# tiberiu44/TTS-Cube

Measured on AMD Instinct MI355X. Metric: audio samples/sec (HiFi-GAN vocoder inference), higher is better.
Workload: dtype f32 (split fp16 hi/lo x3 MFMA, fp32 accumulate)

## Files before the change

### ttscube_amd/csrc/conv1d.hip

```cpp
#include <cmath>
#include <cstdlib>
#include <type_traits>

#include "common.hpp"
#include "conv_kernels.hpp"

namespace ttsc {

template <int C, int K, int D>
__global__ __launch_bounds__(256, 2) void conv_f16x3_wide_kernel(ConvArgs a) {
    extern __shared__ __attribute__((aligned(16))) char smem_raw[];
    constexpr int WM = 2, WN = 2;
    constexpr int MI = 2, NJ = 4, NT = WN * NJ * 32;
    constexpr int SPAN = NT + (K - 1) * D;
    constexpr int SPANP = (SPAN + 63) & ~63;
    constexpr int BUFSZ = 4 * SPAN + 2;
    constexpr int NCHUNK = C / 16, COTN = C / 32;
    constexpr int AITEMS = WM * MI * 2 * 64;
    half8* Xp = reinterpret_cast<half8*>(smem_raw);
    half8* Aw = Xp + 2 * BUFSZ;
    const int tid = threadIdx.x, lane = tid & 63, wave = tid >> 6;
    const int wm = wave / WN, wn = wave % WN;
    const int half = lane >> 5, l31 = lane & 31;
    const int b = blockIdx.z;
    const int q0 = blockIdx.x * NT;
    const int lin = a.in_len ? a.in_len[b] : a.Lin;
    if (a.out_len && q0 >= a.out_len[b]) return;
    const int cotg = blockIdx.y * (WM * MI);
#ifdef TTSC_ABLATE
    const unsigned wg_lin = blockIdx.x + gridDim.x * (blockIdx.y + gridDim.y * blockIdx.z);
#endif
    TTSC_STAMP(a, wg_lin, 0);
    TTSC_STAMP_HWID(a, wg_lin, 15);

    f32x16 acc[MI][NJ];
    const float* ai_first = a.acc_init ? (a.resid ? a.resid : (a.accumulate ? a.y : nullptr)) : nullptr;
    const float* ai_second = (a.acc_init && a.resid && a.accumulate) ? a.y : nullptr;
    const unsigned ai_L = (unsigned)a.Lout;
    const unsigned ai_row0 = ((unsigned)b * a.Cout + (cotg + wm * MI) * 32 + 4 * half) * ai_L;
    const int ai_qw = q0 + wn * (NJ * 32) + l31;
    auto acc_load_first = [&](int i) __attribute__((always_inline)) {
        if (ai_first) {
#pragma unroll
            for (int n = 0; n < NJ; ++n) {
                const int q = ai_qw + n * 32;
                const unsigned o = ai_row0 + (unsigned)(i * 32) * ai_L + (unsigned)(q < a.Lout ? q : 0);
#pragma unroll
                for (int g = 0; g < 4; ++g) {
                    unsigned og = o + (unsigned)(8 * g) * ai_L;
#pragma unroll
                    for (int e = 0; e < 4; ++e) {
                        acc[i][n][4 * g + e] = ai_first[og];
                        og += ai_L;
                    }
                }
            }
        } else {
#pragma unroll
            for (int n = 0; n < NJ; ++n)
#pragma unroll
                for (int r = 0; r < 16; ++r) acc[i][n][r] = 0.f;
        }
    };
    auto acc_init_finish = [&]() __attribute__((always_inline)) {
        const float inv = 1.f / a.w_unscale;
        if (ai_second) {
#pragma unroll
            for (int i = 0; i < MI; ++i)
#pragma unroll
                for (int n0 = 0; n0 < NJ; n0 += 2) {
                    float t[2][16];
#pragma unroll
                    for (int n = 0; n < 2; ++n) {
                        const int q = ai_qw + (n0 + n) * 32;
                        const unsigned o = ai_row0 + (unsigned)(i * 32) * ai_L + (unsigned)(q < a.Lout ? q : 0);
#pragma unroll
                        for (int r = 0; r < 16; ++r) t[n][r] = ai_second[o + (unsigned)((r & 3) + 8 * (r >> 2)) * ai_L];
                    }
#pragma unroll
                    for (int n = 0; n < 2; ++n)
#pragma unroll
                        for (int r = 0; r < 16; ++r) acc[i][n0 + n][r] += t[n][r];
                }
        }
        if (a.bias) {
#pragma unroll
            for (int i = 0; i < MI; ++i) {
                float bv[16];
#pragma unroll
                for (int r = 0; r < 16; ++r) bv[r] = a.bias[(cotg + wm * MI + i) * 32 + (r & 3) + 8 * (r >> 2) + 4 * half];
#pragma unroll
                for (int n = 0; n < NJ; ++n)
#pragma unroll
                    for (int r = 0; r < 16; ++r) acc[i][n][r] += bv[r];
            }
        }
#pragma unroll
        for (int i = 0; i < MI; ++i)
#pragma unroll
            for (int n = 0; n < NJ; ++n)
#pragma unroll
                for (int r = 0; r < 16; ++r) acc[i][n][r] *= inv;
    };
    if (a.acc_init) {
    } else if (a.epi_prefetch && a.bias && (a.resid || a.accumulate)) {
        const float inv = 1.f / a.w_unscale;
#pragma unroll
        for (int i = 0; i < MI; ++i)
#pragma unroll
            for (int r = 0; r < 16; ++r) {
                const float bv = a.bias[(cotg + wm * MI + i) * 32 + (r & 3) + 8 * (r >> 2) + 4 * half] * inv;
#pragma unroll
                for (int j = 0; j < NJ; ++j) acc[i][j][r] = bv;
            }
    } else {
#pragma unroll
        for (int i = 0; i < MI; ++i)
#pragma unroll
            for (int j = 0; j < NJ; ++j)
#pragma unroll
                for (int r = 0; r < 16; ++r) acc[i][j][r] = 0.f;
    }

    const float* xb = a.x + (size_t)b * C * a.Lin;
    const int lo = q0 - D * ((K - 1) / 2);
    const half8* wsrc = reinterpret_cast<const half8*>(a.wph) + (size_t)cotg * 128 + lane;
    if (a.skew) {
        const unsigned lin_id = blockIdx.x + gridDim.x * (blockIdx.y + gridDim.y * blockIdx.z);
        if (lin_id >= 256u && lin_id < 512u)
            for (int z = 0; z < a.skew; ++z) __builtin_amdgcn_s_sleep(127);
    }

    auto stage_A = [&](int c, int j, int slot) __attribute__((always_inline)) {
        if (TTSC_DBG(a, 8)) return;
        const half8* wj = wsrc + (size_t)(j * NCHUNK + c) * (COTN * 128);
#pragma unroll
        for (int i = 0; i < AITEMS / 64 / 4; ++i) {
            const int blk = wave + i * 4;
            __builtin_amdgcn_global_load_lds((const __attribute__((address_space(1))) void*)(wj + blk * 64),
                                             (__attribute__((address_space(3))) void*)(Aw + slot * AITEMS + blk * 64), 16, 0, 0);
        }
    };

    constexpr int XIT = (2 * SPANP + 255) / 256;
    static_assert(XIT <= K, "one staging item per tap");
    float xr[XIT][8];
    unsigned xoff[XIT];
    int xslot[XIT];
    bool xok[XIT];
#pragma unroll
    for (int e = 0; e < XIT; ++e) {
        const int i = tid + e * 256;
        const int h = i >= SPANP ? 1 : 0;
        const int p = i - h * SPANP;
        const int pos = lo + p;
        xok[e] = pos >= 0 && pos < lin;
        int pc = pos > lin - 1 ? lin - 1 : pos;
        pc = pc < 0 ? 0 : pc;
        xoff[e] = (unsigned)(h * 8 * a.Lin + pc);
        xslot[e] = (p < SPAN && i < 2 * SPANP) ? (h * 2) * SPAN + p : 4 * SPAN;
    }
    auto x_issue_item = [&](int e, int c) __attribute__((always_inline)) {
        const float* rc = xb + (size_t)(c * 16) * a.Lin;
#pragma unroll
        for (int ch = 0; ch < 8; ++ch) xr[e][ch] = rc[(size_t)ch * a.Lin + xoff[e]];
    };
    auto x_commit_item = [&](int e, half8* buf) __attribute__((always_inline)) {
        typedef unsigned u32x4 __attribute__((ext_vector_type(4)));
        u32x4 uh, ul;
#pragma unroll
        for (int ch = 0; ch < 8; ch += 2) {
            float v0 = xok[e] ? xr[e][ch] * a.in_scale : 0.f, v1 = xok[e] ? xr[e][ch + 1] * a.in_scale : 0.f;
            v0 = fmaxf(v0, v0 * a.in_slope);
            v1 = fmaxf(v1, v1 * a.in_slope);
            unsigned h, l;
            split2_f16(v0, v1, h, l);
            uh[ch >> 1] = h;
            ul[ch >> 1] = l;
        }
        const half8 vh = __builtin_bit_cast(half8, uh), vl = __builtin_bit_cast(half8, ul);
        buf[xslot[e]] = vh;
        buf[xslot[e] + (xslot[e] < 4 * SPAN ? SPAN : 1)] = vl;
    };

    const half8* xbase = Xp + (unsigned)((half * 2) * SPAN + wn * (NJ * 32) + l31);
    const half8* abase = Aw + (unsigned)(wm * (MI * 128) + lane);
    auto chunk = [&](int c, auto buf_tag, auto par_tag) __attribute__((always_inline)) {
        constexpr int BUF = decltype(buf_tag)::value;
        constexpr int PAR = decltype(par_tag)::value;
        half8* nxt = Xp + (1 - BUF) * BUFSZ;
#pragma unroll
        for (int j = 0; j < K; ++j) {
            const int slot = (PAR + j) & 1;
            if (j + 1 < K)
                stage_A(c, j + 1, slot ^ 1);
            else
                stage_A(c + 1 < NCHUNK ? c + 1 : c, 0, slot ^ 1);
            __builtin_amdgcn_sched_barrier(0);
            half8 ah[MI], al[MI], bh[NJ], bl[NJ];
#pragma unroll
            for (int i = 0; i < MI; ++i) {
                ah[i] = abase[slot * AITEMS + i * 128];
                al[i] = abase[slot * AITEMS + i * 128 + 64];
            }
#pragma unroll
            for (int n = 0; n < NJ; ++n) {
                bh[n] = xbase[BUF * BUFSZ + j * D + n * 32];
                bl[n] = xbase[BUF * BUFSZ + SPAN + j * D + n * 32];
            }
            const int e = K - 1 - j;
            if (e < XIT && !TTSC_DBG(a, 1)) {
                x_commit_item(e, nxt);
                x_issue_item(e, c + 2 < NCHUNK ? c + 2 : NCHUNK - 1);
            }
#pragma unroll
            for (int i = 0; i < MI; ++i)
#pragma unroll
                for (int n = 0; n < NJ; ++n) acc[i][n] = __builtin_amdgcn_mfma_f32_32x32x16_f16(al[i], bh[n], acc[i][n], 0, 0, 0);
#pragma unroll
            for (int i = 0; i < MI; ++i)
#pragma unroll
                for (int n = 0; n < NJ; ++n) acc[i][n] = __builtin_amdgcn_mfma_f32_32x32x16_f16(ah[i], bl[n], acc[i][n], 0, 0, 0);
#pragma unroll
            for (int i = 0; i < MI; ++i)
#pragma unroll
                for (int n = 0; n < NJ; ++n) acc[i][n] = __builtin_amdgcn_mfma_f32_32x32x16_f16(ah[i], bh[n], acc[i][n], 0, 0, 0);
            __builtin_amdgcn_sched_barrier(0);
            if (!TTSC_DBG(a, 2)) __syncthreads();
        }
    };

    stage_A(0, 0, 0);
#pragma unroll
    for (int e = 0; e < XIT; ++e) x_issue_item(e, 0);
    if (a.acc_init) {
        __builtin_amdgcn_sched_barrier(0);
        acc_load_first(0);
        __builtin_amdgcn_sched_barrier(0);
    }
#pragma unroll
    for (int e = 0; e < XIT; ++e) x_commit_item(e, Xp);
#pragma unroll
    for (int e = 0; e < XIT; ++e) x_issue_item(e, 1);
    if (a.acc_init) {
        __builtin_amdgcn_sched_barrier(0);
#pragma unroll
        for (int i = 1; i < MI; ++i) acc_load_first(i);
        acc_init_finish();
    }
    __syncthreads();
    TTSC_STAMP(a, wg_lin, 1);
    for (int c = 0; c < NCHUNK; c += 2) {
        chunk(c, std::integral_constant<int, 0>(), std::integral_constant<int, 0>());
        chunk(c + 1, std::integral_constant<int, 1>(), std::integral_constant<int, (K & 1)>());
    }
// ... 308 lines not shown
                const int ci = c0 + c < a.Cin ? c0 + c : a.Cin - 1;
                const float* row = xb + (size_t)ci * a.Lin;
#pragma unroll
                for (int k = 0; k < PER; ++k) {
                    int pos = lo + tid + k * 256;
                    pos = pos < 0 ? 0 : (pos > a.Lin - 1 ? a.Lin - 1 : pos);
                    v[c][k] = row[pos];
                }
            }
#pragma unroll
            for (int c = 0; c < CH; ++c)
#pragma unroll
                for (int k = 0; k < PER; ++k) {
                    const int p = tid + k * 256, pos = lo + p;
                    float t = v[c][k] * a.in_scale;
                    t = fmaxf(t, t * a.in_slope);
                    if (p < NT + 2 * HALO) xs[c][p] = (c0 + c < a.Cin && pos >= 0 && pos < lin) ? t : 0.f;
                }
        }
        __syncthreads();
        const int nc = a.Cin - c0 < CH ? a.Cin - c0 : CH;
        for (int c = 0; c < nc; ++c) {
            float w[20];
#pragma unroll
            for (int v4 = 0; v4 < 5; ++v4) {
                const f32x4 t = *reinterpret_cast<const f32x4*>(&xs[c][4 * tid + 4 * v4]);
                w[4 * v4] = t[0]; w[4 * v4 + 1] = t[1]; w[4 * v4 + 2] = t[2]; w[4 * v4 + 3] = t[3];
            }
            const float* wk = ws + (c0 + c) * K;
#pragma unroll
            for (int j = 0; j < 16; ++j) {
                if (j < K) {
                    const float wj = wk[j];
#pragma unroll
                    for (int e = 0; e < 4; ++e) acc[e] = fmaf(wj, w[e + j], acc[e]);
                }
            }
        }
    }
    const float bv = a.bias ? a.bias[0] : 0.f;
    float* yb = a.y + (size_t)b * a.Lout;
    const float* rb = a.resid ? a.resid + (size_t)b * a.Lout : nullptr;
    const int q = q0 + 4 * tid;
    float res[4];
#pragma unroll
    for (int e = 0; e < 4; ++e) {
        const bool ok = q + e < a.Lout;
        float t = (acc[e] + bv + (rb && ok ? rb[q + e] : 0.f)) * a.out_scale;
        t = apply_act(t, a.out_act);
        res[e] = t + (a.accumulate && ok ? yb[q + e] : 0.f);
    }
    if (a.nf_flag) {
        bool bad = false;
#pragma unroll
        for (int e = 0; e < 4; ++e) bad = bad || (q + e < a.Lout && !(fabsf(res[e]) <= 3.0e38f));
        if (bad) atomicOr(a.nf_flag, 1u);
    }
    if (q + 3 < a.Lout && (((uintptr_t)(yb + q)) & 15) == 0) {
        const f32x4 o = {res[0], res[1], res[2], res[3]};
        *reinterpret_cast<f32x4*>(yb + q) = o;
    } else {
#pragma unroll
        for (int e = 0; e < 4; ++e)
            if (q + e < a.Lout) yb[q + e] = res[e];
    }
}

template <int MI, int NJ, int TMAX>
static int launch_f16_t(const ConvArgs& a, int B, hipStream_t s) {
    constexpr int NT = 4 * NJ * 32;
    constexpr int MT = MI * 32;
    dim3 grid((unsigned)ceil_div(a.q_cnt, NT), (unsigned)(a.CoutP / MT), (unsigned)B);
    const size_t lds = (size_t)a.span_pad * 4 * 16 + (size_t)a.ntaps * MI * 2 * 64 * 16;
    if (int rc = ensure_full_lds((const void*)conv_f16x3_kernel<MI, NJ, TMAX>)) return rc;
    hipLaunchKernelGGL((conv_f16x3_kernel<MI, NJ, TMAX>), grid, dim3(256), lds, s, a);
    hipError_t e = hipGetLastError();
    if (e != hipSuccess) {
        set_error("conv_f16x3_kernel launch failed: %s", hipGetErrorString(e));
        return TTSC_EHIP;
    }
    return TTSC_OK;
}

template <int C, int K, int D>
static int launch_f16_wide(const ConvArgs& a0, int B, hipStream_t s) {
    constexpr int NT = 256;
    constexpr int SPAN = NT + (K - 1) * D;
    dim3 grid((unsigned)ceil_div(a0.Lout, NT), (unsigned)(C / 128), (unsigned)B);
    ConvArgs a = a0;
    static const int skew_env = getenv("TTSC_CONV_SKEW") ? atoi(getenv("TTSC_CONV_SKEW")) : 0;
    a.skew = ((size_t)grid.x * grid.y * grid.z >= 1024) ? skew_env : 0;
    static const int epi_env = getenv("TTSC_CONV_EPI_PREFETCH") ? atoi(getenv("TTSC_CONV_EPI_PREFETCH")) : 1;
    a.epi_prefetch = (epi_env && !a.gate && a.out_act == TTSC_ACT_NONE && a.Cout == C && (size_t)B * C * a.Lout < (1ull << 32)) ? 1 : 0;
    constexpr size_t lds = (size_t)2 * (4 * SPAN + 2) * 16 + (size_t)2 * (2 * 2 * 2 * 64) * 16;
    if (int rc = ensure_full_lds((const void*)conv_f16x3_wide_kernel<C, K, D>)) return rc;
    hipLaunchKernelGGL((conv_f16x3_wide_kernel<C, K, D>), grid, dim3(256), lds, s, a);
    hipError_t e = hipGetLastError();
    if (e != hipSuccess) {
        set_error("conv_f16x3_wide_kernel launch failed: %s", hipGetErrorString(e));
        return TTSC_EHIP;
    }
    return TTSC_OK;
}


template <int CIN, int J, int MI, int NJ>
__global__ __launch_bounds__(256, 2) void conv_f16x3_tall_kernel(ConvArgs a) {
    extern __shared__ __attribute__((aligned(16))) char smem_raw[];
    constexpr int WM = 2, WN = 2, NT = WN * NJ * 32;
    constexpr int SPAN = NT + (J - 1);
    constexpr int SPANP = (SPAN + 63) & ~63;
    constexpr int BUFSZ = 4 * SPAN + 2;
    constexpr int NCHUNK = CIN / 16;
    constexpr int AITEMS = WM * MI * 2 * 64;
    static_assert(J % 2 == 0 && NCHUNK % 2 == 0, "slot parity: an even number of taps per chunk, chunks in pairs");
    half8* Xp = reinterpret_cast<half8*>(smem_raw);
    half8* Aw = Xp + 2 * BUFSZ;
    const int tid = threadIdx.x, lane = tid & 63, wave = tid >> 6;
    const int wm = wave / WN, wn = wave % WN;
    const int half = lane >> 5, l31 = lane & 31;
    int bx, by, bz;
    if (a.swz_nx > 0) {
        const unsigned id = blockIdx.x, xcd = id & 7u, u = id >> 3;
        by = (int)(u % (unsigned)a.swz_ny);
        const unsigned t = (u / (unsigned)a.swz_ny) * 8u + xcd;
        bx = (int)(t % (unsigned)a.swz_nx);
        bz = (int)(t / (unsigned)a.swz_nx);
        if (bz >= a.fold_B) return;
    } else {
        bx = blockIdx.x, by = blockIdx.y, bz = blockIdx.z;
    }
    const int b = bz;
    const int q0 = a.q_lo + bx * NT;
    const int lin = a.in_len ? a.in_len[b] : a.Lin;
    if (a.out_len && (long)q0 * a.out_stride + a.out_off >= a.out_len[b]) return;
    const int cotg = by * (WM * MI);
    const int cotN = a.CoutP >> 5;

    f32x16 acc[MI][NJ];
#pragma unroll
    for (int i = 0; i < MI; ++i)
#pragma unroll
        for (int j = 0; j < NJ; ++j)
#pragma unroll
            for (int r = 0; r < 16; ++r) acc[i][j][r] = 0.f;

    const float* xb = a.x + (size_t)b * CIN * a.Lin;
    const int lo = q0 - (J - 1);
    const half8* wsrc = reinterpret_cast<const half8*>(a.wph) + (size_t)cotg * 128 + lane;
    auto stage_A = [&](int c, int j, int slot) __attribute__((always_inline)) {
        const half8* wj = wsrc + (size_t)(j * NCHUNK + c) * ((size_t)cotN * 128);
#pragma unroll
        for (int i = 0; i < AITEMS / 64 / 4; ++i) {
            const int blk = wave + i * 4;
            __builtin_amdgcn_global_load_lds((const __attribute__((address_space(1))) void*)(wj + blk * 64),
                                             (__attribute__((address_space(3))) void*)(Aw + slot * AITEMS + blk * 64), 16, 0, 0);
        }
    };
    constexpr int XIT = (2 * SPANP + 255) / 256;
    static_assert(XIT <= J, "one staging item per tap");
    float xr[XIT][8];
    unsigned xoff[XIT];
    int xslot[XIT];
    bool xok[XIT];
#pragma unroll
    for (int e = 0; e < XIT; ++e) {
        const int i = tid + e * 256;
        const int h = i >= SPANP ? 1 : 0;
        const int p = i - h * SPANP;
        const int pos = lo + p;
        xok[e] = pos >= 0 && pos < lin;
        int pc = pos > lin - 1 ? lin - 1 : pos;
        pc = pc < 0 ? 0 : pc;
        xoff[e] = (unsigned)(h * 8 * a.Lin + pc);
        xslot[e] = (p < SPAN && i < 2 * SPANP) ? (h * 2) * SPAN + p : 4 * SPAN;
    }
    auto x_issue_item = [&](int e, int c) __attribute__((always_inline)) {
        const float* rc = xb + (size_t)(c * 16) * a.Lin;
#pragma unroll
        for (int ch = 0; ch < 8; ++ch) xr[e][ch] = rc[(size_t)ch * a.Lin + xoff[e]];
    };
    auto x_commit_item = [&](int e, half8* buf) __attribute__((always_inline)) {
        typedef unsigned u32x4 __attribute__((ext_vector_type(4)));
        u32x4 uh, ul;
#pragma unroll
        for (int ch = 0; ch < 8; ch += 2) {
            float v0 = xok[e] ? xr[e][ch] * a.in_scale : 0.f, v1 = xok[e] ? xr[e][ch + 1] * a.in_scale : 0.f;
            v0 = fmaxf(v0, v0 * a.in_slope);
            v1 = fmaxf(v1, v1 * a.in_slope);
            unsigned h, l;
            split2_f16(v0, v1, h, l);
            uh[ch >> 1] = h;
            ul[ch >> 1] = l;
        }
        const half8 vh = __builtin_bit_cast(half8, uh), vl = __builtin_bit_cast(half8, ul);
        buf[xslot[e]] = vh;
        buf[xslot[e] + (xslot[e] < 4 * SPAN ? SPAN : 1)] = vl;
    };
    const half8* xbase = Xp + (unsigned)((half * 2) * SPAN + wn * (NJ * 32) + l31);
    const half8* abase = Aw + (unsigned)(wm * (MI * 128) + lane);
    auto chunk = [&](int c, auto buf_tag) __attribute__((always_inline)) {
        constexpr int BUF = decltype(buf_tag)::value;
        half8* nxt = Xp + (1 - BUF) * BUFSZ;
#pragma unroll
        for (int j = 0; j < J; ++j) {
            const int slot = j & 1;
            if (j + 1 < J)
                stage_A(c, j + 1, slot ^ 1);
            else
                stage_A(c + 1 < NCHUNK ? c + 1 : c, 0, slot ^ 1);
            __builtin_amdgcn_sched_barrier(0);
            half8 ah[MI], al[MI], bh[NJ], bl[NJ];
#pragma unroll
            for (int i = 0; i < MI; ++i) {
                ah[i] = abase[slot * AITEMS + i * 128];
                al[i] = abase[slot * AITEMS + i * 128 + 64];
            }
#pragma unroll
            for (int n = 0; n < NJ; ++n) {
                bh[n] = xbase[BUF * BUFSZ + (J - 1 - j) + n * 32];
                bl[n] = xbase[BUF * BUFSZ + SPAN + (J - 1 - j) + n * 32];
            }
            const int e = J - 1 - j;
            if (e < XIT) {
                x_commit_item(e, nxt);
                x_issue_item(e, c + 2 < NCHUNK ? c + 2 : NCHUNK - 1);
            }
#pragma unroll
            for (int i = 0; i < MI; ++i)
#pragma unroll
                for (int n = 0; n < NJ; ++n) acc[i][n] = __builtin_amdgcn_mfma_f32_32x32x16_f16(al[i], bh[n], acc[i][n], 0, 0, 0);
#pragma unroll
            for (int i = 0; i < MI; ++i)
#pragma unroll
                for (int n = 0; n < NJ; ++n) acc[i][n] = __builtin_amdgcn_mfma_f32_32x32x16_f16(ah[i], bl[n], acc[i][n], 0, 0, 0);
#pragma unroll
            for (int i = 0; i < MI; ++i)
#pragma unroll
                for (int n = 0; n < NJ; ++n) acc[i][n] = __builtin_amdgcn_mfma_f32_32x32x16_f16(ah[i], bh[n], acc[i][n], 0, 0, 0);
            __builtin_amdgcn_sched_barrier(0);
            __syncthreads();
        }
    };
    stage_A(0, 0, 0);
#pragma unroll
    for (int e = 0; e < XIT; ++e) x_issue_item(e, 0);
#pragma unroll
    for (int e = 0; e < XIT; ++e) x_commit_item(e, Xp);
#pragma unroll
    for (int e = 0; e < XIT; ++e) x_issue_item(e, 1);
    __syncthreads();
    for (int c = 0; c < NCHUNK; c += 2) {
        chunk(c, std::integral_constant<int, 0>());
        chunk(c + 1, std::integral_constant<int, 1>());
    }
    const int q_hi = a.q_lo + a.q_cnt;
#pragma unroll
    for (int i = 0; i < MI; ++i) {
#pragma unroll
        for (int n = 0; n < NJ; ++n) {
            const int q = q0 + wn * (NJ * 32) + n * 32 + l31;
            int cb = (cotg + wm * MI + i) * 32;
            const int r = cb / a.vphase;
            cb -= r * a.vphase;
            const long oo = (long)q * a.out_stride + a.out_off + r;
            const bool ok = (q < q_hi) && (oo >= 0) && (oo < a.Lout) && (r < a.out_stride);
            epilogue_tile(acc[i][n], a, b, cb, oo, ok, half, a.w_unscale);
        }
    }
}

template <int CIN, int J, int MI, int NJ>
static int launch_f16_tall(const ConvArgs& a0, int B, hipStream_t s) {
    constexpr int NT = 2 * NJ * 32, SPAN = NT + (J - 1), MT = 2 * MI * 32;
    ConvArgs a = a0;
    dim3 grid((unsigned)ceil_div(a.q_cnt, NT), (unsigned)(a.CoutP / MT), (unsigned)B);
    static const int swz_env = getenv("TTSC_TALL_SWIZZLE") ? atoi(getenv("TTSC_TALL_SWIZZLE")) : 1;
    if (swz_env && grid.y > 1) {
        a.swz_nx = (int)grid.x;
        a.swz_ny = (int)grid.y;
        a.fold_B = B;
        const unsigned tiles = (unsigned)round_up((int64_t)grid.x * B, 8);
        grid = dim3(tiles * grid.y, 1, 1);
    }
    constexpr size_t lds = (size_t)2 * (4 * SPAN + 2) * 16 + (size_t)2 * (2 * MI * 2 * 64) * 16;
    if (int rc = ensure_full_lds((const void*)conv_f16x3_tall_kernel<CIN, J, MI, NJ>)) return rc;
    hipLaunchKernelGGL((conv_f16x3_tall_kernel<CIN, J, MI, NJ>), grid, dim3(256), lds, s, a);
    hipError_t e = hipGetLastError();
    if (e != hipSuccess) {
        set_error("conv_f16x3_tall_kernel launch failed: %s", hipGetErrorString(e));
        return TTSC_EHIP;
    }
    return TTSC_OK;
}

template <int C, int K>
static int launch_f16_wide_d(const ConvArgs& a, int B, int d, hipStream_t s) {
    if (d == 1) return launch_f16_wide<C, K, 1>(a, B, s);
    if (d == 3) return launch_f16_wide<C, K, 3>(a, B, s);
    return launch_f16_wide<C, K, 5>(a, B, s);
}

template <int C>
static int launch_f16_wide_k(const ConvArgs& a, int B, int d, hipStream_t s) {
    if (a.ntaps == 3) return launch_f16_wide_d<C, 3>(a, B, d, s);
#ifdef TTSC_PROBE_EVENK
    if (a.ntaps == 4) return launch_f16_wide<C, 4, 1>(a, B, s);
    if (a.ntaps == 6) return launch_f16_wide<C, 6, 1>(a, B, s);
#endif
    if (a.ntaps == 7) return launch_f16_wide_d<C, 7>(a, B, d, s);
    return launch_f16_wide_d<C, 11>(a, B, d, s);
}

template <int MI, int NJ>
static int launch_f16(const ConvArgs& a, int B, hipStream_t s) {
    if (a.ntaps <= 3) return launch_f16_t<MI, NJ, 3>(a, B, s);
    if (a.ntaps <= 7) return launch_f16_t<MI, NJ, 7>(a, B, s);
    if (a.ntaps <= 11) return launch_f16_t<MI, NJ, 11>(a, B, s);
    return launch_f16_t<MI, NJ, 16>(a, B, s);
}

template <int MI, int NJ, int WM, int WN>
static int launch_cfg(const ConvArgs& a, int B, hipStream_t s) {
    constexpr int NT = WN * NJ * 32;
    constexpr int MT = WM * MI * 32;
    dim3 grid((unsigned)ceil_div(a.q_cnt, NT), (unsigned)(a.CoutP / MT), (unsigned)B);
    dim3 block(WM * WN * 64);
    size_t lds = (size_t)2 * KC * a.span_pad * sizeof(float);
    TTSC_REQUIRE(lds <= 160 * 1024, "conv_mfma_kernel: receptive field too large for LDS (%zu bytes)", lds);
    if (lds > 64 * 1024)
        if (int rc = ensure_full_lds(reinterpret_cast<const void*>(conv_mfma_kernel<MI, NJ, WM, WN>))) return rc;
    hipLaunchKernelGGL((conv_mfma_kernel<MI, NJ, WM, WN>), grid, block, lds, s, a);
    hipError_t e = hipGetLastError();
    if (e != hipSuccess) {
        set_error("conv_mfma_kernel launch failed: %s", hipGetErrorString(e));
        return TTSC_EHIP;
    }
    return TTSC_OK;
}

static int pick_mt(int Cout) {
    int best = 32, best_pad = (int)round_up(Cout, 32);
    for (int mt : {64, 128}) {
        int pad = (int)round_up(Cout, mt);
        if (pad <= best_pad) {
            best = mt;
            best_pad = pad;
        }
    }
    return best;
}

}

using namespace ttsc;

#include "conv_internal.hpp"

extern "C" int ttsc_conv1d_create(const ttsc_conv1d_cfg* cfg, ttsc_conv1d** out) {
    TTSC_REQUIRE(cfg && out, "ttsc_conv1d_create: null argument");
    TTSC_REQUIRE(cfg->in_channels > 0 && cfg->out_channels > 0 && cfg->kernel_size > 0,
                 "ttsc_conv1d_create: bad channels/kernel (%d,%d,%d)", cfg->in_channels, cfg->out_channels,
                 cfg->kernel_size);
    TTSC_REQUIRE(cfg->stride >= 1 && cfg->dilation >= 1 && cfg->padding >= 0, "ttsc_conv1d_create: bad stride/dilation/padding");
    if (cfg->transposed) {
        TTSC_REQUIRE(cfg->dilation == 1, "ttsc_conv1d_create: ConvTranspose1d supports dilation 1 only");
    } else {
        TTSC_REQUIRE(cfg->stride == 1, "ttsc_conv1d_create: Conv1d supports stride 1 only");
    }
    const int groups = cfg->groups > 1 ? cfg->groups : 1;
    if (groups > 1) {
        TTSC_REQUIRE(!cfg->transposed, "ttsc_conv1d_create: groups need a Conv1d");
        TTSC_REQUIRE(cfg->in_channels % groups == 0 && cfg->out_channels % groups == 0, "ttsc_conv1d_create: channels (%d, %d) not divisible by groups %d",
                     cfg->in_channels, cfg->out_channels, groups);
    }
    ttsc_conv1d* c = new ttsc_conv1d();
// ... 373 lines not shown
extern "C" int ttsc_conv1d_set_nonfinite_flag(ttsc_conv1d* c, uint32_t* flag_dev) {
    TTSC_REQUIRE(c, "ttsc_conv1d_set_nonfinite_flag: null argument");
    c->nf_flag = flag_dev;
    return TTSC_OK;
}

namespace ttsc {
__global__ __launch_bounds__(256) void absmax_kernel(const float* __restrict__ x, long n, unsigned* __restrict__ out) {
    __shared__ float red[4];
    float m = 0.f;
    const long stride = (long)gridDim.x * blockDim.x;
    const long i0 = (long)blockIdx.x * blockDim.x + threadIdx.x;
    if ((reinterpret_cast<uintptr_t>(x) & 15) == 0) {
        const long n4 = n >> 2;
        const float4* x4 = reinterpret_cast<const float4*>(x);
        for (long i = i0; i < n4; i += stride) {
            const float4 v = x4[i];
            m = fmaxf(fmaxf(m, fmaxf(fabsf(v.x), fabsf(v.y))), fmaxf(fabsf(v.z), fabsf(v.w)));
        }
        for (long i = (n4 << 2) + i0; i < n; i += stride) m = fmaxf(m, fabsf(x[i]));
    } else {
        for (long i = i0; i < n; i += stride) m = fmaxf(m, fabsf(x[i]));
    }
#pragma unroll
    for (int off = 32; off >= 1; off >>= 1) m = fmaxf(m, __shfl_xor(m, off));
    if ((threadIdx.x & 63) == 0) red[threadIdx.x >> 6] = m;
    __syncthreads();
    if (threadIdx.x == 0) atomicMax(out, __float_as_uint(fmaxf(fmaxf(red[0], red[1]), fmaxf(red[2], red[3]))));
}
}

extern "C" int ttsc_absmax(const float* x_dev, int64_t n, float* out_dev, void* stream) {
    TTSC_REQUIRE(x_dev && out_dev && n > 0, "ttsc_absmax: bad argument");
    const int blocks = (int)std::min<int64_t>((n / 4 + 255) / 256 + 1, 1024);
    hipLaunchKernelGGL(absmax_kernel, dim3(blocks), dim3(256), 0, (hipStream_t)stream, x_dev, (long)n, reinterpret_cast<unsigned*>(out_dev));
    hipError_t e = hipGetLastError();
    if (e != hipSuccess) {
        set_error("absmax_kernel launch failed: %s", hipGetErrorString(e));
        return TTSC_EHIP;
    }
    return TTSC_OK;
}

extern "C" int ttsc_conv1d_forward_ragged(const ttsc_conv1d* c, const float* x, int32_t B, int64_t Lin, float* y,
                                          const float* resid, const ttsc_conv1d_epilogue* ep, const int32_t* in_len_dev,
                                          const int32_t* out_len_dev, void* stream) {
    return ttsc_conv1d_forward_pitched(c, x, B, Lin, y, resid, ep, in_len_dev, out_len_dev, 0, stream);
}

extern "C" int ttsc_conv1d_forward_pitched(const ttsc_conv1d* c, const float* x, int32_t B, int64_t Lin, float* y,
                                           const float* resid, const ttsc_conv1d_epilogue* ep, const int32_t* in_len_dev,
                                           const int32_t* out_len_dev, int64_t Lout_pitch, void* stream) {
    TTSC_REQUIRE(c && x && y, "ttsc_conv1d_forward: null argument");
    TTSC_REQUIRE(Lout_pitch == 0 || (Lout_pitch > 0 && in_len_dev && out_len_dev),
                 "ttsc_conv1d_forward_pitched: an output pitch needs per-utterance lengths (in_len_dev, out_len_dev)");
    if (!c->has_weight) {
        set_error("ttsc_conv1d_forward: weights not set");
        return TTSC_ESTATE;
    }
    TTSC_REQUIRE(B > 0 && Lin > 0, "ttsc_conv1d_forward: bad B/Lin (%d, %lld)", B, (long long)Lin);
    TTSC_REQUIRE(!ep || (ep->in_slope >= 0.f && ep->in_slope <= 1.f), "ttsc_conv1d_forward: in_slope must be in [0,1]");
    const auto& g = c->cfg;
    const int64_t Lout = Lout_pitch > 0 ? Lout_pitch : ttsc_conv1d_out_len(c, Lin);
    TTSC_REQUIRE(Lout > 0, "ttsc_conv1d_forward: output length %lld <= 0", (long long)Lout);
    TTSC_REQUIRE(Lin < (1ll << 30) && Lout < (1ll << 30), "ttsc_conv1d_forward: length too large");
    hipStream_t s = (hipStream_t)stream;
    for (const auto& ph : c->phases) {
        ConvArgs a;
        a.x = x;
        a.y = y;
        a.resid = resid;
        a.nf_flag = nullptr;
        a.wp = ph.wp_dev;
        a.wph = ph.wph_dev;
        a.w_unscale = c->w_unscale;
        a.bias = (c->dev_weights && c->bias_ext) ? c->bias_ext : c->bias_dev;
        a.in_len = in_len_dev;
        a.out_len = out_len_dev;
        a.dbg = 0;
        a.skew = 0;
        a.acc_init = 0;
        a.epi_prefetch = 0;
        a.swz_nx = a.swz_ny = 0;
        a.fold_S = a.fold_B = 0;
        a.amax_x = a.amax_w = nullptr;
        a.amax_out = nullptr;
#ifdef TTSC_ABLATE
        if (const char* ev = getenv("TTSC_CONV_DBG")) a.dbg = atoi(ev);
        a.prof = nullptr;
        if (const char* ev = getenv("TTSC_PROF_PTR")) a.prof = reinterpret_cast<unsigned long long*>(strtoull(ev, nullptr, 0));
#endif
        a.vphase = c->vfused ? ((c->vrow4 && c->precision == TTSC_PREC_F16X3) ? -4 : g.out_channels) : 0;
        if (a.vphase == -4) {
            TTSC_REQUIRE(!(ep && ep->gate_dev), "ttsc_conv1d_forward: the gate epilogue is not available on this transposed layer");
            TTSC_REQUIRE(((uintptr_t)y % 16 == 0) && (!resid || (uintptr_t)resid % 16 == 0), "ttsc_conv1d_forward: y / resid must be 16-byte aligned for ConvTranspose1d(k=4, s=4)");
        }
        a.Cin = c->groups > 1 ? c->cin_tile : g.in_channels;
        a.CinTot = g.in_channels;
        a.groups = c->groups;
        a.cin_g = c->cin_g;
        a.cout_g = c->cout_g;
        a.CinP = c->CinP;
        a.Cout = g.out_channels;
        a.CoutP = c->CoutP;
        a.Lin = (int)Lin;
        a.Lout = (int)Lout;
        a.ntaps = ph.ntaps;
        a.tap_base = ph.tap_base;
        a.tap_step = ph.tap_step;
        a.out_stride = ph.out_stride;
        a.out_off = ph.out_off;
        if (!g.transposed) {
            a.q_lo = 0;
            a.q_cnt = (int)Lout;
        } else if (c->vfused) {
            int64_t qlo = -floor_div((g.stride - 1) - g.padding, g.stride);
            int64_t qhi = floor_div(Lout - 1 + g.padding, g.stride) + 1;
            if (qhi <= qlo) continue;
            a.q_lo = (int)qlo;
            a.q_cnt = (int)(qhi - qlo);
        } else {
            int64_t qlo = -floor_div(ph.r - g.padding, g.stride);
            int64_t qhi = floor_div(Lout - 1 - ph.r + g.padding, g.stride) + 1;
            if (qhi <= qlo) continue;
            a.q_lo = (int)qlo;
            a.q_cnt = (int)(qhi - qlo);
        }
        const int last = (ph.ntaps - 1) * ph.tap_step;
        a.min_shift = ph.tap_base + (last < 0 ? last : 0);
        a.span = c->NT + (last < 0 ? -last : last);
        a.span_pad = a.span + 1;
        a.in_scale = ep ? ep->in_scale : 1.f;
        const float* w_plain = c->dev_weights ? c->w_plain_ext : c->w_plain_dev;
        const bool use_cout1 = !g.transposed && c->groups == 1 && g.out_channels == 1 && g.in_channels <= 64 && g.kernel_size <= 16 && g.dilation == 1 &&
                               w_plain && !(ep && ep->gate_dev);
        if (c->precision == TTSC_PREC_F16X3 && !use_cout1) {
            a.in_scale *= c->act_scale;
            a.w_unscale = c->w_unscale / c->act_scale;
        }
        a.in_slope = ep ? ep->in_slope : 1.f;
        a.out_scale = ep ? ep->out_scale : 1.f;
        a.out_act = ep ? ep->out_act : TTSC_ACT_NONE;
        a.accumulate = ep ? ep->accumulate : 0;
        a.gate = ep ? ep->gate_dev : nullptr;
        a.gate_slope = ep ? ep->gate_slope : 1.f;
        int rc;
        if (use_cout1) {
            a.wp = w_plain;
            a.nf_flag = c->nf_flag;
            dim3 grid((unsigned)ceil_div(Lout, 1024), (unsigned)B);
            hipLaunchKernelGGL(conv_cout1_kernel, grid, dim3(256), 0, s, a);
            hipError_t e = hipGetLastError();
            if (e != hipSuccess) {
                set_error("conv_cout1_kernel launch failed: %s", hipGetErrorString(e));
                return TTSC_EHIP;
            }
            rc = TTSC_OK;
        } else if (c->precision == TTSC_PREC_F16X3) {
            const int nt = c->MT >= 64 ? 256 : 512;
            a.span = nt + (last < 0 ? -last : last);
            a.span_pad = a.span;
            TTSC_REQUIRE(ph.ntaps <= 16, "f16x3 path supports at most 16 taps per phase (got %d)", ph.ntaps);
            auto wgs16 = [&](int mt, int nt) { return (long)ceil_div(a.q_cnt, nt) * (c->CoutP / mt) * B; };
            auto set_nt16 = [&](int n) {
                a.span = n + (last < 0 ? -last : last);
                a.span_pad = a.span;
            };
            static const bool big_only = getenv("TTSC_F16_TILE") && atoi(getenv("TTSC_F16_TILE")) == 0;
            const char* wide_ev = getenv("TTSC_CONV_WIDE");
            const int wide_env = wide_ev ? atoi(wide_ev) : 1;
            const long want16 = 512;
            const bool wide_shape = !g.transposed && !a.gate && g.in_channels == g.out_channels &&
                                    (g.out_channels == 128 || g.out_channels == 256) &&
                                    ((g.kernel_size == 3 || g.kernel_size == 7 || g.kernel_size == 11)
#ifdef TTSC_PROBE_EVENK
                                     || ((g.kernel_size == 4 || g.kernel_size == 6) && g.dilation == 1)
#endif
                                     ) &&
                                    (g.dilation == 1 || g.dilation == 3 || g.dilation == 5) &&
                                    g.padding == g.dilation * (g.kernel_size - 1) / 2;
            static const int acc_init_env = getenv("TTSC_CONV_ACC_INIT") ? atoi(getenv("TTSC_CONV_ACC_INIT")) : 1;
            a.acc_init = (acc_init_env && wide_env && wide_shape && a.out_act == TTSC_ACT_NONE && a.out_scale == 1.f && c->CoutP == g.out_channels &&
                          (size_t)B * g.out_channels * Lout < (1ull << 32)) ? 1 : 0;
            static const bool tall_on = !(getenv("TTSC_CONV_TALL") && atoi(getenv("TTSC_CONV_TALL")) == 0);
            const bool tall0 = g.in_channels == 512 && ph.ntaps == 4 && c->CoutP % 256 == 0;
            const bool tall1 = g.in_channels == 256 && ph.ntaps == 6 && c->CoutP % 128 == 0;
            const bool tall_shape = tall_on && c->vfused && a.vphase > 0 && !a.gate && c->CinP == g.in_channels && (tall0 || tall1);
            if (tall_shape && (wide_env == 2 || (long)ceil_div(a.q_cnt, tall0 ? 128 : 256) * (c->CoutP / (tall0 ? 256 : 128)) * B >= want16)) {
                rc = tall0 ? launch_f16_tall<512, 4, 4, 2>(a, B, s) : launch_f16_tall<256, 6, 2, 4>(a, B, s);
            } else if (wide_env && wide_shape && (wide_env == 2 || (long)ceil_div(a.Lout, 256) * (g.out_channels / 128) * B >= want16)) {
                if (g.out_channels == 256)
                    rc = launch_f16_wide_k<256>(a, B, g.dilation, s);
                else
                    rc = launch_f16_wide_k<128>(a, B, g.dilation, s);
            } else if (c->MT >= 64) {
                if (big_only || wgs16(64, 256) >= want16)
                    rc = launch_f16<2, 2>(a, B, s);
                else if (wgs16(64, 128) >= want16) {
                    set_nt16(128);
                    rc = launch_f16<2, 1>(a, B, s);
                } else {
                    set_nt16(128);
                    rc = launch_f16<1, 1>(a, B, s);
                }
            } else {
                if (big_only || wgs16(32, 512) >= want16)
                    rc = launch_f16<1, 4>(a, B, s);
                else if (wgs16(32, 256) >= want16) {
                    set_nt16(256);
                    rc = launch_f16<1, 2>(a, B, s);
                } else {
                    set_nt16(128);
                    rc = launch_f16<1, 1>(a, B, s);
                }
            }
        } else {
            auto wgs = [&](int mt, int nt) { return (long)ceil_div(a.q_cnt, nt) * (c->CoutP / mt) * B; };
            auto set_nt = [&](int nt) {
                a.span = nt + (last < 0 ? -last : last);
                a.span_pad = a.span + 1;
            };
            static const long want_env = getenv("TTSC_CONV_WANT") ? atol(getenv("TTSC_CONV_WANT")) : 512;
            static const int narrow_env = getenv("TTSC_CONV_NARROW") ? atoi(getenv("TTSC_CONV_NARROW")) : 1;
            const long want = want_env;
            auto padded = [&](int nt) { return (long)ceil_div(a.q_cnt, nt) * nt; };
            auto narrower_pays = [&](int nt_big, int nt_small) { return narrow_env && padded(nt_small) * 8 < padded(nt_big) * 7; };
            if (c->MT == 128) {
                if (wgs(128, 128) >= want && !narrower_pays(128, 64)) { set_nt(128); rc = launch_cfg<2, 2, 2, 2>(a, B, s); }
                else if (wgs(64, 128) >= want && !narrower_pays(128, 64)) { set_nt(128); rc = launch_cfg<1, 2, 2, 2>(a, B, s); }
                else { set_nt(64); rc = launch_cfg<1, 1, 2, 2>(a, B, s); }
            } else if (c->MT == 64) {
                if (wgs(64, 256) >= want && !narrower_pays(256, 128)) { set_nt(256); rc = launch_cfg<2, 2, 1, 4>(a, B, s); }
                else if (wgs(64, 128) >= want && !narrower_pays(128, 64)) { set_nt(128); rc = launch_cfg<1, 2, 2, 2>(a, B, s); }
                else { set_nt(64); rc = launch_cfg<1, 1, 2, 2>(a, B, s); }
            } else {
                if (wgs(32, 512) >= want && !narrower_pays(512, 256)) { set_nt(512); rc = launch_cfg<1, 4, 1, 4>(a, B, s); }
                else if (wgs(32, 256) >= want && !narrower_pays(256, 128)) { set_nt(256); rc = launch_cfg<1, 2, 1, 4>(a, B, s); }
                else { set_nt(128); rc = launch_cfg<1, 1, 1, 4>(a, B, s); }
            }
        }
        if (rc) return rc;
    }
    return TTSC_OK;
}


extern "C" int ttsc_respair_supported(const ttsc_conv1d* c1, const ttsc_conv1d* c2) {
    if (!c1 || !c2) return 0;
    const auto &g1 = c1->cfg, &g2 = c2->cfg;
    const int k = g1.kernel_size;
    if (g1.transposed || g2.transposed) return 0;
    if (g1.in_channels != 32 || g1.out_channels != 32 || g2.in_channels != 32 || g2.out_channels != 32) return 0;
    if (g2.kernel_size != k || !(k == 3 || k == 7 || k == 11)) return 0;
    if (g2.dilation != 1 || g2.padding != (k - 1) / 2 || g1.padding != g1.dilation * (k - 1) / 2) return 0;
    if ((k - 1) * g1.dilation > 64) return 0;
    if (c1->precision != TTSC_PREC_F16X3 || c2->precision != TTSC_PREC_F16X3) return 0;
    if (!c1->has_weight || !c2->has_weight || !c1->bias_dev || !c2->bias_dev) return 0;
    return 1;
}

extern "C" int ttsc_respair_forward(const ttsc_conv1d* c1, const ttsc_conv1d* c2, const float* x, int32_t B, int64_t L, float* y,
                                    int32_t accumulate, const int32_t* len_dev, void* stream) {
    TTSC_REQUIRE(c1 && c2 && x && y, "ttsc_respair_forward: null argument");
    TTSC_REQUIRE(ttsc_respair_supported(c1, c2), "ttsc_respair_forward: this pair of layers is not eligible for the fused kernel");
    TTSC_REQUIRE(x != y, "ttsc_respair_forward: y must not alias x");
    TTSC_REQUIRE(B > 0 && L > 0 && L < (1ll << 30), "ttsc_respair_forward: bad B/L");
    PairArgs a;
    a.x = x;
    a.y = y;
    a.w1 = c1->phases[0].wph_dev;
// ... 33 lines not shown
```

### ttscube_amd/csrc/conv_kernels.hpp

```cpp
#pragma once
#include "common.hpp"
#include "conv_internal.hpp"

namespace ttsc {

typedef float f32x16 __attribute__((ext_vector_type(16)));

#ifdef TTSC_ABLATE
#define TTSC_DBG(args, bit) (((args).dbg & (bit)) != 0)
#define TTSC_STAMP(args, wg, i)                                                                              \
    do {                                                                                                     \
        if ((args).prof && threadIdx.x == 0) (args).prof[(size_t)(wg) * 24 + (i)] = __builtin_amdgcn_s_memrealtime(); \
    } while (0)
#define TTSC_STAMP_HWID(args, wg, i)                                                                         \
    do {                                                                                                     \
        if ((args).prof && threadIdx.x == 0) {                                                               \
            unsigned hw, xcc;                                                                                \
            asm volatile("s_getreg_b32 %0, hwreg(HW_REG_HW_ID)" : "=s"(hw));                                 \
            asm volatile("s_getreg_b32 %0, hwreg(HW_REG_XCC_ID)" : "=s"(xcc));                               \
            (args).prof[(size_t)(wg) * 24 + (i)] = ((unsigned long long)(xcc & 0xf) << 32) | hw;            \
        }                                                                                                    \
    } while (0)
#else
#define TTSC_DBG(args, bit) false
#define TTSC_STAMP(args, wg, i) do {} while (0)
#define TTSC_STAMP_HWID(args, wg, i) do {} while (0)
#endif

static constexpr int KC = 16;

struct ConvArgs {
    const float* x;
    float* y;
    const float* resid;
    const float* wp;
    const void* wph;
    float w_unscale;
    const float* bias;
    const int* in_len;
    const int* out_len;
    int Cin, CinP, Cout, CoutP;
    int CinTot;
    int groups, cin_g, cout_g;
    int Lin, Lout;
    int ntaps, tap_base, tap_step;
    int out_stride, out_off;
    int q_lo, q_cnt;
    int span, span_pad, min_shift;
    float in_scale, in_slope, out_scale;
    int out_act, accumulate;
    int vphase;
    int acc_init;
    int epi_prefetch;
    int swz_nx, swz_ny;
    int skew;
    int dbg;
#ifdef TTSC_ABLATE
    unsigned long long* prof;
#endif
    unsigned* nf_flag;
    const float* gate;
    float gate_slope;
    int fold_S, fold_B;
    const float* amax_x;
    const float* amax_w;
    unsigned* amax_out;
};

__device__ __forceinline__ float pow2_to(float m, int target) {
    const int ex = (int)((__float_as_uint(m) >> 23) & 0xffu);
    if (ex == 0 || ex == 255) return 1.f;
    int s = target - (ex - 126);
    s = s > 100 ? 100 : (s < -100 ? -100 : s);
    return __uint_as_float((unsigned)(127 + s) << 23);
}
int launch_amax2(const float* x, long nx, float* out_x, const float* w, long nw, float* out_w, hipStream_t s, bool prezeroed = false);
static constexpr int SPLIT_X_TARGET = 15, SPLIT_W_TARGET = 10;

__device__ __forceinline__ float apply_act(float v, int act) {
    if (act == TTSC_ACT_TANH) return tanhf(v);
    if (act == TTSC_ACT_RELU) return fmaxf(v, 0.f);
    if (act == TTSC_ACT_SIGMOID) return 1.f / (1.f + expf(-v));
    return v;
}

__device__ __forceinline__ void epilogue_tile(const f32x16& acc, const ConvArgs& a, int b, int co_base, long o, bool qok,
                                              int half, float acc_scale, float* amax_acc = nullptr) {
    const long o_c = qok ? o : 0;
#pragma unroll
    for (int g = 0; g < 4; ++g) {
        float rv[4], yv[4], bv[4], res[4];
        size_t idx[4];
#pragma unroll
        for (int e = 0; e < 4; ++e) {
            const int co = co_base + 8 * g + 4 * half + e;
            const int co_c = co < a.Cout ? co : a.Cout - 1;
            idx[e] = ((size_t)b * a.Cout + co_c) * a.Lout + o_c;
        }
        if (a.bias) {
#pragma unroll
            for (int e = 0; e < 4; ++e) {
                const int co = co_base + 8 * g + 4 * half + e;
                bv[e] = a.bias[co < a.Cout ? co : a.Cout - 1];
            }
        } else {
#pragma unroll
            for (int e = 0; e < 4; ++e) bv[e] = 0.f;
        }
        if (a.resid) {
#pragma unroll
            for (int e = 0; e < 4; ++e) rv[e] = a.resid[idx[e]];
        } else {
#pragma unroll
            for (int e = 0; e < 4; ++e) rv[e] = 0.f;
        }
        if (a.accumulate) {
#pragma unroll
            for (int e = 0; e < 4; ++e) yv[e] = a.y[idx[e]];
        } else {
#pragma unroll
            for (int e = 0; e < 4; ++e) yv[e] = 0.f;
        }
        if (a.gate) {
            float gv[4];
#pragma unroll
            for (int e = 0; e < 4; ++e) gv[e] = a.gate[idx[e]];
#pragma unroll
            for (int e = 0; e < 4; ++e)
                res[e] = ((acc[4 * g + e] * acc_scale + bv[e]) * (gv[e] > 0.f ? 1.f : a.gate_slope) + rv[e]) * a.out_scale + yv[e];
        } else if (a.out_act == TTSC_ACT_NONE) {
#pragma unroll
            for (int e = 0; e < 4; ++e) res[e] = (acc[4 * g + e] * acc_scale + bv[e] + rv[e]) * a.out_scale + yv[e];
        } else {
#pragma unroll
            for (int e = 0; e < 4; ++e) res[e] = apply_act((acc[4 * g + e] * acc_scale + bv[e] + rv[e]) * a.out_scale, a.out_act) + yv[e];
        }
#pragma unroll
// ... 471 lines not shown
```

Before: 287.5 million.

## Add lean buffer-load path and shortened tap loop for tall transposed convs

Adds a LEAN template variant to the wide and tall f16x3 conv kernels. It loads inputs through buffer resources with out-of-bounds offsets that return zero, instead of clamped global loads plus per-element masking. The tall kernel also gains a tap-count parameter so output-channel tiles at or beyond short_from run J-1 taps, skipping a tap that is structurally zero for those polyphase outputs. Lean is on by default when the input size fits in 32-bit byte offsets and the input scale is positive. This doubles the template instantiations and relies on buffer OOB semantics and the short_from calculation being correct.

```diff
diff --git a/ttscube_amd/csrc/conv1d.hip b/ttscube_amd/csrc/conv1d.hip
--- a/ttscube_amd/csrc/conv1d.hip
+++ b/ttscube_amd/csrc/conv1d.hip
@@ -1,3 +1,4 @@
+#include <climits>
 #include <cmath>
 #include <cstdlib>
 #include <type_traits>
@@ -7,7 +8,12 @@
 
 namespace ttsc {
 
-template <int C, int K, int D>
+static constexpr unsigned LEAN_OOB = 0x80000000u;
+__device__ __forceinline__ float lean_load(__amdgpu_buffer_rsrc_t rs, unsigned voff, int soff) {
+    return __uint_as_float(__builtin_amdgcn_raw_buffer_load_b32(rs, (int)voff, soff, 0));
+}
+
+template <int C, int K, int D, bool LEAN>
 __global__ __launch_bounds__(256, 2) void conv_f16x3_wide_kernel(ConvArgs a) {
     extern __shared__ __attribute__((aligned(16))) char smem_raw[];
     constexpr int WM = 2, WN = 2;
@@ -159,18 +165,27 @@
         pc = pc < 0 ? 0 : pc;
         xoff[e] = (unsigned)(h * 8 * a.Lin + pc);
         xslot[e] = (p < SPAN && i < 2 * SPANP) ? (h * 2) * SPAN + p : 4 * SPAN;
-    }
+        if (LEAN) xoff[e] = (xok[e] && xslot[e] < 4 * SPAN) ? xoff[e] * 4u : LEAN_OOB;
+    }
+    const __amdgpu_buffer_rsrc_t xrs = __builtin_amdgcn_make_buffer_rsrc(const_cast<float*>(xb), 0, LEAN ? C * a.Lin * 4 : 0, 0x00020000);
+    const int xrow = a.Lin * 4;
     auto x_issue_item = [&](int e, int c) __attribute__((always_inline)) {
-        const float* rc = xb + (size_t)(c * 16) * a.Lin;
-#pragma unroll
-        for (int ch = 0; ch < 8; ++ch) xr[e][ch] = rc[(size_t)ch * a.Lin + xoff[e]];
+        if constexpr (LEAN) {
+            const int s0 = c * 16 * xrow;
+#pragma unroll
+            for (int ch = 0; ch < 8; ++ch) xr[e][ch] = lean_load(xrs, xoff[e], s0 + ch * xrow);
+        } else {
+            const float* rc = xb + (size_t)(c * 16) * a.Lin;
+#pragma unroll
+            for (int ch = 0; ch < 8; ++ch) xr[e][ch] = rc[(size_t)ch * a.Lin + xoff[e]];
+        }
     };
     auto x_commit_item = [&](int e, half8* buf) __attribute__((always_inline)) {
         typedef unsigned u32x4 __attribute__((ext_vector_type(4)));
         u32x4 uh, ul;
 #pragma unroll
         for (int ch = 0; ch < 8; ch += 2) {
-            float v0 = xok[e] ? xr[e][ch] * a.in_scale : 0.f, v1 = xok[e] ? xr[e][ch + 1] * a.in_scale : 0.f;
+            float v0 = (LEAN || xok[e]) ? xr[e][ch] * a.in_scale : 0.f, v1 = (LEAN || xok[e]) ? xr[e][ch + 1] * a.in_scale : 0.f;
             v0 = fmaxf(v0, v0 * a.in_slope);
             v1 = fmaxf(v1, v1 * a.in_slope);
             unsigned h, l;
@@ -645,8 +660,8 @@
     return TTSC_OK;
 }
 
-template <int C, int K, int D>
-static int launch_f16_wide(const ConvArgs& a0, int B, hipStream_t s) {
+template <int C, int K, int D, bool LEAN>
+static int launch_f16_wide_l(const ConvArgs& a0, int B, hipStream_t s) {
     constexpr int NT = 256;
     constexpr int SPAN = NT + (K - 1) * D;
     dim3 grid((unsigned)ceil_div(a0.Lout, NT), (unsigned)(C / 128), (unsigned)B);
@@ -656,8 +671,8 @@
     static const int epi_env = getenv("TTSC_CONV_EPI_PREFETCH") ? atoi(getenv("TTSC_CONV_EPI_PREFETCH")) : 1;
     a.epi_prefetch = (epi_env && !a.gate && a.out_act == TTSC_ACT_NONE && a.Cout == C && (size_t)B * C * a.Lout < (1ull << 32)) ? 1 : 0;
     constexpr size_t lds = (size_t)2 * (4 * SPAN + 2) * 16 + (size_t)2 * (2 * 2 * 2 * 64) * 16;
-    if (int rc = ensure_full_lds((const void*)conv_f16x3_wide_kernel<C, K, D>)) return rc;
-    hipLaunchKernelGGL((conv_f16x3_wide_kernel<C, K, D>), grid, dim3(256), lds, s, a);
+    if (int rc = ensure_full_lds((const void*)conv_f16x3_wide_kernel<C, K, D, LEAN>)) return rc;
+    hipLaunchKernelGGL((conv_f16x3_wide_kernel<C, K, D, LEAN>), grid, dim3(256), lds, s, a);
     hipError_t e = hipGetLastError();
     if (e != hipSuccess) {
         set_error("conv_f16x3_wide_kernel launch failed: %s", hipGetErrorString(e));
@@ -666,8 +681,13 @@
     return TTSC_OK;
 }
 
-
-template <int CIN, int J, int MI, int NJ>
+template <int C, int K, int D>
+static int launch_f16_wide(const ConvArgs& a, int B, hipStream_t s) {
+    return a.lean ? launch_f16_wide_l<C, K, D, true>(a, B, s) : launch_f16_wide_l<C, K, D, false>(a, B, s);
+}
+
+
+template <int CIN, int J, int MI, int NJ, bool LEAN>
 __global__ __launch_bounds__(256, 2) void conv_f16x3_tall_kernel(ConvArgs a) {
     extern __shared__ __attribute__((aligned(16))) char smem_raw[];
     constexpr int WM = 2, WN = 2, NT = WN * NJ * 32;
@@ -676,7 +696,7 @@
     constexpr int BUFSZ = 4 * SPAN + 2;
     constexpr int NCHUNK = CIN / 16;
     constexpr int AITEMS = WM * MI * 2 * 64;
-    static_assert(J % 2 == 0 && NCHUNK % 2 == 0, "slot parity: an even number of taps per chunk, chunks in pairs");
+    static_assert(NCHUNK % 2 == 0, "slot parity: chunks in pairs (two chunks of NTAPS taps each end on the slot they started on)");
     half8* Xp = reinterpret_cast<half8*>(smem_raw);
     half8* Aw = Xp + 2 * BUFSZ;
     const int tid = threadIdx.x, lane = tid & 63, wave = tid >> 6;
@@ -711,11 +731,12 @@
     const float* xb = a.x + (size_t)b * CIN * a.Lin;
     const int lo = q0 - (J - 1);
     const half8* wsrc = reinterpret_cast<const half8*>(a.wph) + (size_t)cotg * 128 + lane;
+    const int wave_s = LEAN ? __builtin_amdgcn_readfirstlane(wave) : wave;
     auto stage_A = [&](int c, int j, int slot) __attribute__((always_inline)) {
         const half8* wj = wsrc + (size_t)(j * NCHUNK + c) * ((size_t)cotN * 128);
 #pragma unroll
         for (int i = 0; i < AITEMS / 64 / 4; ++i) {
-            const int blk = wave + i * 4;
+            const int blk = wave_s + i * 4;
             __builtin_amdgcn_global_load_lds((const __attribute__((address_space(1))) void*)(wj + blk * 64),
                                              (__attribute__((address_space(3))) void*)(Aw + slot * AITEMS + blk * 64), 16, 0, 0);
         }
@@ -737,18 +758,27 @@
         pc = pc < 0 ? 0 : pc;
         xoff[e] = (unsigned)(h * 8 * a.Lin + pc);
         xslot[e] = (p < SPAN && i < 2 * SPANP) ? (h * 2) * SPAN + p : 4 * SPAN;
-    }
+        if (LEAN) xoff[e] = (xok[e] && xslot[e] < 4 * SPAN) ? xoff[e] * 4u : LEAN_OOB;
+    }
+    const __amdgpu_buffer_rsrc_t xrs = __builtin_amdgcn_make_buffer_rsrc(const_cast<float*>(xb), 0, LEAN ? CIN * a.Lin * 4 : 0, 0x00020000);
+    const int xrow = a.Lin * 4;
     auto x_issue_item = [&](int e, int c) __attribute__((always_inline)) {
-        const float* rc = xb + (size_t)(c * 16) * a.Lin;
-#pragma unroll
-        for (int ch = 0; ch < 8; ++ch) xr[e][ch] = rc[(size_t)ch * a.Lin + xoff[e]];
+        if constexpr (LEAN) {
+            const int s0 = c * 16 * xrow;
+#pragma unroll
+            for (int ch = 0; ch < 8; ++ch) xr[e][ch] = lean_load(xrs, xoff[e], s0 + ch * xrow);
+        } else {
+            const float* rc = xb + (size_t)(c * 16) * a.Lin;
+#pragma unroll
+            for (int ch = 0; ch < 8; ++ch) xr[e][ch] = rc[(size_t)ch * a.Lin + xoff[e]];
+        }
     };
     auto x_commit_item = [&](int e, half8* buf) __attribute__((always_inline)) {
         typedef unsigned u32x4 __attribute__((ext_vector_type(4)));
         u32x4 uh, ul;
 #pragma unroll
         for (int ch = 0; ch < 8; ch += 2) {
-            float v0 = xok[e] ? xr[e][ch] * a.in_scale : 0.f, v1 = xok[e] ? xr[e][ch + 1] * a.in_scale : 0.f;
+            float v0 = (LEAN || xok[e]) ? xr[e][ch] * a.in_scale : 0.f, v1 = (LEAN || xok[e]) ? xr[e][ch + 1] * a.in_scale : 0.f;
             v0 = fmaxf(v0, v0 * a.in_slope);
             v1 = fmaxf(v1, v1 * a.in_slope);
             unsigned h, l;
@@ -762,13 +792,16 @@
     };
     const half8* xbase = Xp + (unsigned)((half * 2) * SPAN + wn * (NJ * 32) + l31);
     const half8* abase = Aw + (unsigned)(wm * (MI * 128) + lane);
-    auto chunk = [&](int c, auto buf_tag) __attribute__((always_inline)) {
+    auto chunk = [&](int c, auto buf_tag, auto par_tag, auto ntaps_tag) __attribute__((always_inline)) {
         constexpr int BUF = decltype(buf_tag)::value;
+        constexpr int PAR = decltype(par_tag)::value;
+        constexpr int NTAPS = decltype(ntaps_tag)::value;
+        static_assert(XIT <= NTAPS, "one staging item per tap");
         half8* nxt = Xp + (1 - BUF) * BUFSZ;
 #pragma unroll
-        for (int j = 0; j < J; ++j) {
-            const int slot = j & 1;
-            if (j + 1 < J)
+        for (int j = 0; j < NTAPS; ++j) {
+            const int slot = (PAR + j) & 1;
+            if (j + 1 < NTAPS)
                 stage_A(c, j + 1, slot ^ 1);
             else
                 stage_A(c + 1 < NCHUNK ? c + 1 : c, 0, slot ^ 1);
@@ -784,7 +817,7 @@
                 bh[n] = xbase[BUF * BUFSZ + (J - 1 - j) + n * 32];
                 bl[n] = xbase[BUF * BUFSZ + SPAN + (J - 1 - j) + n * 32];
             }
-            const int e = J - 1 - j;
+            const int e = NTAPS - 1 - j;
             if (e < XIT) {
                 x_commit_item(e, nxt);
                 x_issue_item(e, c + 2 < NCHUNK ? c + 2 : NCHUNK - 1);
@@ -813,9 +846,16 @@
 #pragma unroll
     for (int e = 0; e < XIT; ++e) x_issue_item(e, 1);
     __syncthreads();
-    for (int c = 0; c < NCHUNK; c += 2) {
-        chunk(c, std::integral_constant<int, 0>());
-        chunk(c + 1, std::integral_constant<int, 1>());
+    if (LEAN && by >= a.short_from) {
+        for (int c = 0; c < NCHUNK; c += 2) {
+            chunk(c, std::integral_constant<int, 0>(), std::integral_constant<int, 0>(), std::integral_constant<int, J - 1>());
+            chunk(c + 1, std::integral_constant<int, 1>(), std::integral_constant<int, ((J - 1) & 1)>(), std::integral_constant<int, J - 1>());
+        }
+    } else {
+        for (int c = 0; c < NCHUNK; c += 2) {
+            chunk(c, std::integral_constant<int, 0>(), std::integral_constant<int, 0>(), std::integral_constant<int, J>());
+            chunk(c + 1, std::integral_constant<int, 1>(), std::integral_constant<int, (J & 1)>(), std::integral_constant<int, J>());
+        }
     }
     const int q_hi = a.q_lo + a.q_cnt;
 #pragma unroll
@@ -833,8 +873,8 @@
     }
 }
 
-template <int CIN, int J, int MI, int NJ>
-static int launch_f16_tall(const ConvArgs& a0, int B, hipStream_t s) {
+template <int CIN, int J, int MI, int NJ, bool LEAN>
+static int launch_f16_tall_l(const ConvArgs& a0, int B, hipStream_t s) {
     constexpr int NT = 2 * NJ * 32, SPAN = NT + (J - 1), MT = 2 * MI * 32;
     ConvArgs a = a0;
     dim3 grid((unsigned)ceil_div(a.q_cnt, NT), (unsigned)(a.CoutP / MT), (unsigned)B);
@@ -847,14 +887,19 @@
         grid = dim3(tiles * grid.y, 1, 1);
     }
     constexpr size_t lds = (size_t)2 * (4 * SPAN + 2) * 16 + (size_t)2 * (2 * MI * 2 * 64) * 16;
-    if (int rc = ensure_full_lds((const void*)conv_f16x3_tall_kernel<CIN, J, MI, NJ>)) return rc;
-    hipLaunchKernelGGL((conv_f16x3_tall_kernel<CIN, J, MI, NJ>), grid, dim3(256), lds, s, a);
+    if (int rc = ensure_full_lds((const void*)conv_f16x3_tall_kernel<CIN, J, MI, NJ, LEAN>)) return rc;
+    hipLaunchKernelGGL((conv_f16x3_tall_kernel<CIN, J, MI, NJ, LEAN>), grid, dim3(256), lds, s, a);
     hipError_t e = hipGetLastError();
     if (e != hipSuccess) {
         set_error("conv_f16x3_tall_kernel launch failed: %s", hipGetErrorString(e));
         return TTSC_EHIP;
     }
     return TTSC_OK;
+}
+
+template <int CIN, int J, int MI, int NJ>
+static int launch_f16_tall(const ConvArgs& a, int B, hipStream_t s) {
+    return a.lean ? launch_f16_tall_l<CIN, J, MI, NJ, true>(a, B, s) : launch_f16_tall_l<CIN, J, MI, NJ, false>(a, B, s);
 }
 
 template <int C, int K>
@@ -1394,6 +1439,8 @@
         a.acc_init = 0;
         a.epi_prefetch = 0;
         a.swz_nx = a.swz_ny = 0;
+        a.lean = 0;
+        a.short_from = INT_MAX;
         a.fold_S = a.fold_B = 0;
         a.amax_x = a.amax_w = nullptr;
         a.amax_out = nullptr;
@@ -1498,6 +1545,9 @@
             const bool tall0 = g.in_channels == 512 && ph.ntaps == 4 && c->CoutP % 256 == 0;
             const bool tall1 = g.in_channels == 256 && ph.ntaps == 6 && c->CoutP % 128 == 0;
             const bool tall_shape = tall_on && c->vfused && a.vphase > 0 && !a.gate && c->CinP == g.in_channels && (tall0 || tall1);
+            const char* lean_ev = getenv("TTSC_CONV_LEAN");
+            a.lean = (!(lean_ev && atoi(lean_ev) == 0) && (int64_t)g.in_channels * Lin * 4 < (1ll << 31) && a.in_scale > 0.f && std::isfinite(a.in_scale)) ? 1 : 0;
+            if (tall_shape && (tall0 ? 256 : 128) == g.out_channels) a.short_from = g.kernel_size - (ph.ntaps - 1) * g.stride;
             if (tall_shape && (wide_env == 2 || (long)ceil_div(a.q_cnt, tall0 ? 128 : 256) * (c->CoutP / (tall0 ? 256 : 128)) * B >= want16)) {
                 rc = tall0 ? launch_f16_tall<512, 4, 4, 2>(a, B, s) : launch_f16_tall<256, 6, 2, 4>(a, B, s);
             } else if (wide_env && wide_shape && (wide_env == 2 || (long)ceil_div(a.Lout, 256) * (g.out_channels / 128) * B >= want16)) {
diff --git a/ttscube_amd/csrc/conv_kernels.hpp b/ttscube_amd/csrc/conv_kernels.hpp
--- a/ttscube_amd/csrc/conv_kernels.hpp
+++ b/ttscube_amd/csrc/conv_kernels.hpp
@@ -53,6 +53,8 @@
     int acc_init;
     int epi_prefetch;
     int swz_nx, swz_ny;
+    int lean;
+    int short_from;
     int skew;
     int dbg;
 #ifdef TTSC_ABLATE
```

Measured after the change: 290.5 million, median of 6. 1.0% higher.
